# emsig/emg3d

Hardware: AMD Instinct MI355X
Metric: Mcells*smoother-iters/s (fp64) per multigrid cycle (higher is better)
Workload: dtype c128 (complex fp64)

## Files before the change

emg3d_amd/_cycle.py:

```python
import os

import numpy as np
import torch

from emg3d_amd import _lib

__all__ = ['run_cycles', 'coarse_correction', 'coarse_schedule', 'smooth_level', 'stop_reason',
           'ConvergenceError', 'current_sc_dir', 'current_lr_dir']


class ConvergenceError(Exception):
    """Multigrid as preconditioner diverged or stagnated: aborts the Krylov solver."""


def current_sc_dir(sc_dir, grid):
    kept = tuple(n % 2 != 0 or n < 3 or sc_dir == axis + 1 for axis, n in enumerate(grid.shape_cells))
    codes = {(0, 0, 0): 0, (1, 0, 0): 1, (0, 1, 0): 2, (0, 0, 1): 3, (0, 1, 1): 4, (1, 0, 1): 5, (1, 1, 0): 6,
             (1, 1, 1): 6}
    return codes[tuple(int(k) for k in kept)]


_LR_AXES = {0: (), 1: (1,), 2: (2,), 3: (3,), 4: (2, 3), 5: (1, 3), 6: (1, 2), 7: (1, 2, 3)}
_LR_CODE = {axes: code for code, axes in _LR_AXES.items()}

# ... 56 lines not shown
    return budget


class CoarseCorrection:

    def __init__(self, first, first_level, var):
        self.var = var
        self.levels = {first_level: first}

    def run(self, steps):
        var = self.var
        loud = var.verb > 4
        trace = var.first_cycle and var.verb > 3
        sc_at = {}
        for step in steps:
            kind, level = step[0], step[1]
            lv = self.levels[level]
            if kind == SMOOTH:
                smooth_level(lv, step[2], var.lr_dir, var)
                if loud:
                    _log_smoothing(var, level, lv, step[3], step[4], step[5])
            elif kind == DOWN:
                sc_at[level] = current_sc_dir(var.sc_dir, lv.grid)
                lv.residual(store=True, norm=False)
                self.levels[level + 1] = lv.restrict_to(sc_at[level])
            elif kind == UP:
                lv.prolong_from(sc_at[level])
                if trace:
                    var.level_all.append(level)
            elif trace:
                var.level_all.append(level)


def _log_smoothing(var, level, lv, what, it=0, cycmax=None):
    n = lv.grid.shape_cells
    norm = lv.residual(store=False, norm=True)
    visits = var.cycmax if cycmax is None else cycmax
    var.cprint(f"     {it:2} {level} {visits} [{n[0]:3}, {n[1]:3}, {n[2]:3}]: {norm:.3e} {what}", 4)


USE_GRAPHS = os.environ.get('EMG3D_AMD_GRAPHS', '1') != '0'
GRAPH_AFTER = int(os.environ.get('EMG3D_AMD_GRAPH_AFTER', '2'))
CONCURRENT = 0


def coarse_correction(clv, var, budget, first_level=1, graphed=None, top=None):
    depth = int(var.clevel[var.sc_dir])
    steps = coarse_schedule(var.cycle, var.cycmax, depth, first_level, budget, var.nu_pre, var.nu_coarse,
# ... 202 lines not shown
    if leave is not None:
        leave()


def _can_switch(top):
    try:
        top.reserve_residual_equation()
    except torch.cuda.OutOfMemoryError:
        return False
    return True


def _one_cycle(top, var, it, loud):
    if var.clevel[var.sc_dir] == 0:
        smooth_level(top, var.nu_coarse, var.lr_dir, var)
        if loud:
            _log_smoothing(var, 0, top, "coarsest level", it, 1)
        return
    if var.nu_pre > 0:
        smooth_level(top, var.nu_pre, var.lr_dir, var)
        if loud:
            _log_smoothing(var, 0, top, "pre-smoothing", it)
    sc = current_sc_dir(var.sc_dir, top.grid)
    top.residual(store=True, norm=False)
    coarse_correction(top.restrict_to(sc), var, var.cycmax, top=top)
    top.prolong_from(sc)
    if var.first_cycle and var.verb > 3:
        var.level_all.append(0)
    if var.nu_post > 0:
        smooth_level(top, var.nu_post, var.lr_dir, var)
        if loud:
            _log_smoothing(var, 0, top, "post-smoothing", it)


def _level0_visits(var):
    return 1 if var.clevel[var.sc_dir] == 0 else var.cycmax
```

emg3d_amd/_device.py:

```python
import ctypes

import numpy as np
import torch

from emg3d_amd import _lib, meshes
from emg3d_amd import core as _core

_vp = ctypes.c_void_p


def _stream():
    return _vp(torch.cuda.current_stream().cuda_stream)


def _ptr(t, offset_elems=0):
    return _vp(t.data_ptr() + offset_elems * t.element_size())


def coarsen_flags(sc_dir):
    return (sc_dir not in (1, 5, 6), sc_dir not in (2, 4, 6), sc_dir not in (3, 4, 5))


def interp_table(cnodes, nodes):
    i = np.searchsorted(cnodes, nodes) - 1
# ... 388 lines not shown
        for t in tabs:
            pw_slots.append(len(fparts))
            fparts.append(t[1])
        foff = np.cumsum([0] + [a.size for a in fparts])
        fbuf = self.work.upload(np.concatenate(fparts))
        ioff = np.cumsum([0] + [t[0].size for t in tabs])
        ibuf = self.work.upload(np.concatenate([t[0] for t in tabs]))
        wptr = [(_ptr(fbuf, int(foff[i])) if i is not None else None) for i in slots]
        pwptr = [_ptr(fbuf, int(foff[i])) for i in pw_slots]
        ilptr = [_ptr(ibuf, int(ioff[d])) for d in range(3)]
        link = {'level': clevel, 'buffers': (fbuf, ibuf), 'wptr': wptr, 'ilptr': ilptr, 'pwptr': pwptr}
        self.children[sc_dir] = link
        return link

    def restrict_to(self, sc_dir):
        link = self.child(sc_dir)
        c = link['level']
        nx, ny, nz = self.grid.shape_cells
        _lib.check(_lib.lib().emg3d_dev_restrict_clear_batch(
            *c.parts(c.s), *c.parts(c.e), *self.parts(self.r), *link['wptr'], nx, ny, nz, sc_dir,
            self.is_complex, self.batch, self.grid.n_edges, c.grid.n_edges, _stream()), 'emg3d_dev_restrict')
        return c

    def prolong_from(self, sc_dir):
        link = self.children[sc_dir]
        c = link['level']
        nx, ny, nz = self.grid.shape_cells
        _lib.check(_lib.lib().emg3d_dev_prolong_batch(
            *self.parts(self.e), *c.parts(c.e), *link['ilptr'], *link['pwptr'], nx, ny, nz, sc_dir,
            self.is_complex, self.batch, self.grid.n_edges, c.grid.n_edges, _stream()),
            'emg3d_dev_prolong')
```

emg3d_amd/_lib.py:

```python
import ctypes
import os
import subprocess

_HERE = os.path.dirname(os.path.abspath(__file__))
CSRC = os.path.join(_HERE, 'csrc')
LIBDIR = os.path.join(_HERE, 'lib')
LIBPATH = os.path.join(LIBDIR, 'libemg3d_amd.so')
HEADER = os.path.join(os.path.dirname(_HERE), 'include', 'emg3d_amd.h')
SOURCES = [os.path.join(CSRC, f) for f in ('kernels.hip', 'stencil.h', 'launch.h', 'cplx.h', 'receivers.h', 'krylov.h', 'adjoint.h')] + [HEADER]

HIPCC_FLAGS = ['--offload-arch=gfx950', '-O3', '-std=c++17', '-fPIC', '-shared', '-ffp-contract=fast-honor-pragmas']


class Emg3dAmdError(RuntimeError):
    """A C-ABI call returned a non-zero status."""


def build(force=False, verbose=False):
    os.makedirs(LIBDIR, exist_ok=True)
    stale = (not os.path.exists(LIBPATH) or
             any(os.path.getmtime(s) > os.path.getmtime(LIBPATH) for s in SOURCES))
    if force or stale:
        hipcc = os.environ.get('HIPCC', 'hipcc')
        cmd = [hipcc] + HIPCC_FLAGS + [os.path.join(CSRC, 'kernels.hip'), '-o', LIBPATH]
# ... 29 lines not shown
    'emg3d_core_amat_x': (_ci, [_vp] * 13 + [_ci] * 4),
    'emg3d_core_gauss_seidel': (_ci, [_ci] + [_vp] * 13 + [_ci] * 5),
    'emg3d_core_restrict': (_ci, [_vp] * 15 + [_ci] * 5),
    'emg3d_core_blocks_to_amat': (_ci, [_vp] * 5 + [_ci] * 4),
    'emg3d_core_solve': (_ci, [_vp, _vp, _ci, _ci]),
    'emg3d_gs_scratch_bytes': (_sz, [_ci] * 5),
    'emg3d_line_fac_bytes': (_sz, [_ci] * 5),
    'emg3d_line_fac_bytes_lv': (_sz, [ctypes.POINTER(Level), _ci]),
    'emg3d_line_compact_used': (_ci, [ctypes.POINTER(Level), _ci]),
    'emg3d_point_compact_used': (_ci, [ctypes.POINTER(Level)]),
    'emg3d_line_lfac_bytes': (_sz, [_ci] * 4),
    'emg3d_dev_line_setup': (_ci, [ctypes.POINTER(Level), _ci, _vp, _vp, _vp]),
    'emg3d_point_fac_bytes': (_sz, [_ci] * 4),
    'emg3d_point_fac_bytes_lv': (_sz, [ctypes.POINTER(Level)]),
    'emg3d_dev_eta_is_imaginary': (_ci, [ctypes.POINTER(Level), ctypes.POINTER(_ci), _vp]),
    'emg3d_dev_point_setup': (_ci, [ctypes.POINTER(Level), _vp, _vp]),
    'emg3d_dev_gauss_seidel': (_ci, [ctypes.POINTER(Level), _ci, _ci, _vp, _vp, _vp, _sz, _vp]),
    'emg3d_residual_ws_len': (_sz, [_ci] * 3),
    'emg3d_dev_residual': (_ci, [ctypes.POINTER(Level), _vp, _vp, _vp, _vp, _sz, _vp, _vp]),
    'emg3d_dev_restrict': (_ci, [_vp] * 15 + [_ci] * 5 + [_vp]),
    'emg3d_dev_prolong': (_ci, [_vp] * 12 + [_ci] * 5 + [_vp]),
    'emg3d_dev_restrict_batch': (_ci, [_vp] * 15 + [_ci] * 6 + [_sz, _sz, _vp]),
    'emg3d_dev_restrict_clear_batch': (_ci, [_vp] * 18 + [_ci] * 6 + [_sz, _sz, _vp]),
    'emg3d_dev_prolong_batch': (_ci, [_vp] * 12 + [_ci] * 6 + [_sz, _sz, _vp]),
    'emg3d_dev_restrict_param': (_ci, [_vp, _vp] + [_ci] * 5 + [_vp]),
    'emg3d_dev_pec_zero': (_ci, [_vp] * 3 + [_ci] * 4 + [_vp]),
    'emg3d_krylov_ws_len': (_sz, []),
    'emg3d_dev_krylov_step': (_ci, [_sz, _ci, _vp, _ci, _vp, _vp, _vp, _ci, _vp, _vp, _vp, _ci, _vp, _vp, _vp, _sz, _vp]),
    'emg3d_dev_apply_operator': (_ci, [ctypes.POINTER(Level), _vp, _vp, _vp, _vp]),
    'emg3d_dev_zero': (_ci, [_vp, _sz, _vp]),
    'emg3d_dev_copy': (_ci, [_vp, _vp, _sz, _vp]),
    'emg3d_dev_gradient_accumulate': (_ci, [_ci] * 4 + [_vp] * 6 + [ctypes.c_double] * 2 + [_vp] * 5),
    'emg3d_dev_source_field': (_ci, [_ci] * 4 + [_vp] * 7 + [_ci] + [ctypes.c_double] * 2 + [_vp] * 4),
    'emg3d_dev_volume_model': (_ci, [_ci] * 4 + [_vp] * 5 + [_ci] + [_vp] * 3 + [ctypes.c_double] * 4 + [_vp] * 5),
    'emg3d_dev_magnetic_field': (_ci, [_ci] * 4 + [_vp] * 7 + [ctypes.c_double] * 2 + [_vp] * 4),
    'emg3d_dev_spline_filter': (_ci, [_vp] + [_ci] * 4 + [_vp]),
    'emg3d_dev_spline_eval': (_ci, [_vp] + [_ci] * 4 + [_vp, _ci, _vp, _vp]),
    'emg3d_dev_linear_eval': (_ci, [_vp] + [_ci] * 4 + [_vp, _vp, _ci, _vp, _vp]),
    'emg3d_dev_volume_average': (_ci, [_vp] + [_ci] * 3 + [_vp] * 10 + [_ci] * 3 + [_vp, _ci, _vp]),
}

LEVEL_ETA_IMAG = 1
LEVEL_LINE_COMPACT = 2
LEVEL_POINT_COMPACT = 4

_lib = None
# ... 43 lines not shown
```

emg3d_amd/csrc/kernels.hip:

```cpp
#include <hip/hip_runtime.h>

#include <algorithm>
#include <cstdio>
#include <cstdlib>
#include <cstring>
#include <string>
#include <type_traits>

#include "../../include/emg3d_amd.h"
#include "launch.h"

using emg::cplx;

namespace {

thread_local std::string g_err;

int fail(int code, const char *what)
{
    g_err = what;
    return code;
}

int hipfail(hipError_t e, const char *where)
// ... 20 lines not shown
    L.batch = lv->batch > 1 ? lv->batch : 1;
    L.bstride = lv->batch > 1 ? (size_t)lv->batch_stride : 0;
    L.flags = lv->flags;
    return L;
}

using emg::cdiv;
using emg::cnt_par;
using emg::sc_flags;
using emg::ScDirs;

inline dim3 d3(emg::Dim3 d) { return dim3(d.x, d.y, d.z); }

int g_point_slab = 0;
int g_point_tile_min = 1 << 20;
int g_line_fuse = 2;
int g_line_fuse_max = 1 << 30;
int g_skip_repeat = 1;
int g_tile_fuse = 1;
int g_line_lds = 1;
int g_point_prefetch = 0;
int g_residual_zb = 8;
int g_residual_roll = 1;
int g_line_occ2 = 0;
int g_point_small = 512;
int g_line_lpw = 0;
int g_line_stream = 2;
int g_line_order = 1;
int g_line_stream_r = 0;
int g_line_stream_bmin = 64;
int g_line_stream_lf = 1;
int g_line_wide = 33;
int g_line_wide_bt = 0;
int g_line_debug = 0;
int g_line_compact = 0;
int g_line_compact_rd = 0;
int g_line_compact_colour = 1;
constexpr int LS_PROD_COMPACT = 384;

template <class T> bool pst_stored_half(int flags);
template <> bool pst_stored_half<double>(int) { return true; }
template <> bool pst_stored_half<cplx>(int flags) { return (flags & emg::LEVEL_ETA_IMAG) != 0; }
int g_point_compact = 0;
template <class T> int pst_mode(int flags)
{
    const bool compact = g_point_compact > 0 || (g_point_compact == 0 && (flags & emg::LEVEL_POINT_COMPACT));
// ... 1383 lines not shown
    out += blockIdx.x;
    __shared__ double sm[256];
    double acc = 0.0;
    for (int i = threadIdx.x; i < n; i += 256) acc += partial[i];
    sm[threadIdx.x] = acc;
    __syncthreads();
    for (int s = 128; s > 0; s >>= 1) {
        if ((int)threadIdx.x < s) sm[threadIdx.x] += sm[threadIdx.x + s];
        __syncthreads();
    }
    if (threadIdx.x == 0) *out = sm[0];
}

template <class T> __global__ __launch_bounds__(256) void k_restrict(emg::Restrict<T> R)
{
    const int cix = blockIdx.x * blockDim.x + threadIdx.x;
    const int ciy = blockIdx.y * blockDim.y + threadIdx.y;
    const int b = blockIdx.z / R.cnzn, ciz = blockIdx.z - b * R.cnzn;
    if (cix >= R.cnxn || ciy >= R.cnyn) return;
    R.rx += b * R.fstride; R.ry += b * R.fstride; R.rz += b * R.fstride;
    R.crx += b * R.cstride; R.cry += b * R.cstride; R.crz += b * R.cstride;
    if (R.cex) { R.cex += b * R.cstride; R.cey += b * R.cstride; R.cez += b * R.cstride; }
    emg::restrict_node<T>(R, cix, ciy, ciz);
}

template <class T> __global__ __launch_bounds__(256) void k_prolong(emg::Prolong<T> P)
{
    const int ix = blockIdx.x * blockDim.x + threadIdx.x;
    const int iy = blockIdx.y * blockDim.y + threadIdx.y;
    const int b = blockIdx.z / (P.nz + 1), iz = blockIdx.z - b * (P.nz + 1);
    if (ix > P.nx || iy > P.ny) return;
    P.ex += b * P.fstride; P.ey += b * P.fstride; P.ez += b * P.fstride;
    P.cex += b * P.cstride; P.cey += b * P.cstride; P.cez += b * P.cstride;
    emg::prolong_cell<T>(P, ix, iy, iz);
}

template <class T>
__global__ __launch_bounds__(256) void k_restrict_param(T *out, const T *in, int nx, int ny, int cnx,
                                                        int cny, int fx, int fy, int fz)
{
    const int cix = blockIdx.x * blockDim.x + threadIdx.x;
    const int ciy = blockIdx.y * blockDim.y + threadIdx.y;
    const int ciz = blockIdx.z;
    if (cix >= cnx || ciy >= cny) return;
    emg::restrict_param_cell<T>(out, in, nx, ny, cnx, cny, fx, fy, fz, cix, ciy, ciz);
}
// ... 435 lines not shown
    if (sumsq) hipLaunchKernelGGL(k_reduce_sum, dim3(L.batch), dim3(256), 0, st, ws, (int)nblk, sumsq);
    HIP_TRY(hipGetLastError());
    return 0;
}

template <class T>
int launch_restrict(void *crx, void *cry, void *crz, const void *rx, const void *ry, const void *rz,
                    const double *const w[9], int nx, int ny, int nz, int sc_dir, hipStream_t st, int batch = 1,
                    size_t fstride = 0, size_t cstride = 0, void *cex = nullptr, void *cey = nullptr, void *cez = nullptr)
{
    const ScDirs f = sc_flags(sc_dir);
    if ((f.cx && nx % 2) || (f.cy && ny % 2) || (f.cz && nz % 2))
        return fail(EMG3D_ERR_BADARG, "restrict: odd cell count in a coarsened direction");
    emg::Restrict<T> R = emg::make_restrict<T>(crx, cry, crz, rx, ry, rz, w, nx, ny, nz, sc_dir);
    R.batch = batch > 1 ? batch : 1; R.fstride = fstride; R.cstride = cstride;
    R.cex = (T *)cex; R.cey = (T *)cey; R.cez = (T *)cez;
    const emg::Dim3 g = emg::cell_grid(R.cnxn, R.cnyn, R.cnzn);
    hipLaunchKernelGGL(k_restrict<T>, dim3(g.x, g.y, g.z * R.batch), d3(emg::cell_block()), 0, st, R);
    HIP_TRY(hipGetLastError());
    return 0;
}

template <class T>
int launch_prolong(void *ex, void *ey, void *ez, const void *cex, const void *cey, const void *cez,
                   const int32_t *ilx, const int32_t *ily, const int32_t *ilz, const double *wx,
                   const double *wy, const double *wz, int nx, int ny, int nz, int sc_dir, hipStream_t st,
                   int batch = 1, size_t fstride = 0, size_t cstride = 0)
{
    emg::Prolong<T> P =
        emg::make_prolong<T>(ex, ey, ez, cex, cey, cez, ilx, ily, ilz, wx, wy, wz, nx, ny, nz, sc_dir);
    P.batch = batch > 1 ? batch : 1; P.fstride = fstride; P.cstride = cstride;
    const emg::Dim3 g = emg::cell_grid(nx + 1, ny + 1, nz + 1);
    hipLaunchKernelGGL(k_prolong<T>, dim3(g.x, g.y, g.z * P.batch), d3(emg::cell_block()), 0, st, P);
    HIP_TRY(hipGetLastError());
    return 0;
}

template <class T>
int launch_restrict_param(void *out, const void *in, int nx, int ny, int nz, int sc_dir, hipStream_t st)
{
    const ScDirs f = sc_flags(sc_dir);
    const int fx = f.cx ? 2 : 1, fy = f.cy ? 2 : 1, fz = f.cz ? 2 : 1;
    const int cnx = nx / fx, cny = ny / fy, cnz = nz / fz;
    const dim3 block = d3(emg::cell_block());
    const dim3 grid = d3(emg::cell_grid(cnx, cny, cnz));
    hipLaunchKernelGGL(k_restrict_param<T>, grid, block, 0, st, (T *)out, (const T *)in, nx, ny, cnx, cny, fx, fy, fz);
    HIP_TRY(hipGetLastError());
    return 0;
}


struct DevBuf {
    void *d = nullptr;
    size_t bytes = 0;
    ~DevBuf() { if (d) (void)hipFree(d); }
    hipError_t up(const void *h, size_t n)
// ... 49 lines not shown
    hipError_t e = b.up(tmp, sizeof(double) * (size_t)n);
    delete[] tmp;
    return e;
}

}

extern "C" {

int emg3d_version(void) { return EMG3D_AMD_VERSION; }
const char *emg3d_last_error(void) { return g_err.c_str(); }

struct OptionEntry { const char *name; int *value; };
static const OptionEntry g_options[] = {
    {"point_slab", &g_point_slab},       {"point_tile_min", &g_point_tile_min}, {"line_fuse", &g_line_fuse},
    {"line_fuse_max", &g_line_fuse_max}, {"skip_repeat", &g_skip_repeat},       {"tile_fuse", &g_tile_fuse},
    {"line_lds", &g_line_lds},           {"point_prefetch", &g_point_prefetch}, {"residual_zb", &g_residual_zb},
    {"line_occ2", &g_line_occ2},         {"point_small", &g_point_small},       {"line_lpw", &g_line_lpw},
    {"line_debug", &g_line_debug},       {"line_stream", &g_line_stream},       {"line_stream_r", &g_line_stream_r},
    {"line_order", &g_line_order},       {"point_order", &emg::point_order_ref()},
    {"line_stream_bmin", &g_line_stream_bmin}, {"line_stream_lf", &g_line_stream_lf}, {"residual_roll", &g_residual_roll},
    {"line_wide", &g_line_wide},         {"line_wide_bt", &g_line_wide_bt},     {"line_compact", &g_line_compact},
    {"line_compact_rd", &g_line_compact_rd}, {"point_compact", &g_point_compact},
    {"line_compact_colour", &g_line_compact_colour},
};
constexpr int N_OPTIONS = sizeof(g_options) / sizeof(g_options[0]);
static int g_options_generation = 0;

int emg3d_option_count(void) { return N_OPTIONS; }
const char *emg3d_option_name(int i) { return (i >= 0 && i < N_OPTIONS) ? g_options[i].name : nullptr; }

int emg3d_set_option(const char *name, int value)
{
    if (!name) return fail(EMG3D_ERR_BADARG, "set_option: null name");
    if (!std::strcmp(name, "residual_zb") && value < 1) value = 1;
    if (!std::strcmp(name, "line_lpw") && value != 0 && value != 4 && value != 8 && value != 16 && value != 32)
        return fail(EMG3D_ERR_BADARG, "line_lpw: 0, 4, 8, 16 or 32");
    if (!std::strcmp(name, "line_debug") && value != 0 && !std::getenv("EMG3D_AMD_ALLOW_DEBUG"))
        return fail(EMG3D_ERR_BADARG, "line_debug: wrong results by design; set EMG3D_AMD_ALLOW_DEBUG=1 to use it");
    if (!std::strcmp(name, "line_stream_r") && value != 0 && (value < 4 || value > 32 || value % emg::LINE_PAD != 0))
        return fail(EMG3D_ERR_BADARG, "line_stream_r: 0 (= 16) or a multiple of 4 in 4..32");
    if (!std::strcmp(name, "line_wide") && (value < 0 || value > emg::WIDE_N0_MAX)) return fail(EMG3D_ERR_BADARG, "line_wide: 0 .. 64");
    if (!std::strcmp(name, "line_wide_bt") && value != 0 && value != 192 && value != 256) return fail(EMG3D_ERR_BADARG, "line_wide_bt: 0, 192 or 256");
    if (!std::strcmp(name, "line_compact_rd") && value != 0 && value != 4 && value != 8) return fail(EMG3D_ERR_BADARG, "line_compact_rd: 0, 4 or 8");
    if (!std::strcmp(name, "point_compact") && (value < -1 || value > 1)) return fail(EMG3D_ERR_BADARG, "point_compact: -1, 0 or 1");
    if (!std::strcmp(name, "line_compact") && (value < -1 || value > 1)) return fail(EMG3D_ERR_BADARG, "line_compact: -1, 0 or 1");
    if (!std::strcmp(name, "line_order") && (value < 0 || value > 2)) return fail(EMG3D_ERR_BADARG, "line_order: 0, 1 or 2");
    if (!std::strcmp(name, "point_order") && (value < 0 || value > 1)) return fail(EMG3D_ERR_BADARG, "point_order: 0 or 1");
    for (const OptionEntry &o : g_options)
        if (!std::strcmp(name, o.name)) {
            if (*o.value != value) ++g_options_generation;
            *o.value = value;
            return 0;
        }
    return fail(EMG3D_ERR_BADARG, "set_option: unknown option");
}

int emg3d_options_generation(void) { return g_options_generation; }

#ifdef EMG_WIDE_STAMPS
int emg3d_debug_wide_stamps(unsigned long long *out)
{
    return (int)hipMemcpyFromSymbol(out, HIP_SYMBOL(g_wide_stamps), sizeof(unsigned long long) * 32);
}
#endif

const char *emg3d_line_kernel_name(int lr, int nx, int ny, int nz, int is_complex, int batch)
{
    if (lr < 1 || lr > 3 || nx < 2 || ny < 2 || nz < 2) return "";
    const emg::LineClass lc = emg::line_class(lr - 1, nx, ny, nz, 3);
    if (lc.lines <= 0) return "";
// ... 199 lines not shown
{
    if (sc_dir < 0 || sc_dir > 6) return fail(EMG3D_ERR_BADARG, "restrict: sc_dir must be 0..6");
    const double *const w[9] = {wxl, wx0, wxr, wyl, wy0, wyr, wzl, wz0, wzr};
    return is_complex ? launch_restrict<cplx>(crx, cry, crz, rx, ry, rz, w, nx, ny, nz, sc_dir, (hipStream_t)stream, batch,
                                              fine_stride, coarse_stride)
                      : launch_restrict<double>(crx, cry, crz, rx, ry, rz, w, nx, ny, nz, sc_dir, (hipStream_t)stream,
                                                batch, fine_stride, coarse_stride);
}

int emg3d_dev_restrict_clear_batch(void *crx, void *cry, void *crz, void *cex, void *cey, void *cez, const void *rx,
                                   const void *ry, const void *rz, const double *wxl, const double *wx0,
                                   const double *wxr, const double *wyl, const double *wy0, const double *wyr,
                                   const double *wzl, const double *wz0, const double *wzr, int nx, int ny, int nz,
                                   int sc_dir, int is_complex, int batch, size_t fine_stride, size_t coarse_stride,
                                   void *stream)
{
    if (sc_dir < 0 || sc_dir > 6) return fail(EMG3D_ERR_BADARG, "restrict: sc_dir must be 0..6");
    if (!cex || !cey || !cez) return fail(EMG3D_ERR_BADARG, "restrict_clear: coarse field missing");
    const double *const w[9] = {wxl, wx0, wxr, wyl, wy0, wyr, wzl, wz0, wzr};
    return is_complex ? launch_restrict<cplx>(crx, cry, crz, rx, ry, rz, w, nx, ny, nz, sc_dir, (hipStream_t)stream, batch,
                                              fine_stride, coarse_stride, cex, cey, cez)
                      : launch_restrict<double>(crx, cry, crz, rx, ry, rz, w, nx, ny, nz, sc_dir, (hipStream_t)stream,
                                                batch, fine_stride, coarse_stride, cex, cey, cez);
}

int emg3d_dev_prolong_batch(void *ex, void *ey, void *ez, const void *cex, const void *cey, const void *cez,
                            const int32_t *ilx, const int32_t *ily, const int32_t *ilz, const double *wx,
                            const double *wy, const double *wz, int nx, int ny, int nz, int sc_dir, int is_complex,
                            int batch, size_t fine_stride, size_t coarse_stride, void *stream)
{
    if (sc_dir < 0 || sc_dir > 6) return fail(EMG3D_ERR_BADARG, "prolong: sc_dir must be 0..6");
    return is_complex ? launch_prolong<cplx>(ex, ey, ez, cex, cey, cez, ilx, ily, ilz, wx, wy, wz, nx, ny, nz, sc_dir,
                                             (hipStream_t)stream, batch, fine_stride, coarse_stride)
                      : launch_prolong<double>(ex, ey, ez, cex, cey, cez, ilx, ily, ilz, wx, wy, wz, nx, ny, nz, sc_dir,
                                               (hipStream_t)stream, batch, fine_stride, coarse_stride);
}

int emg3d_dev_restrict_param(void *out, const void *in, int nx, int ny, int nz, int sc_dir, int is_complex,
                             void *stream)
{
    if (sc_dir < 0 || sc_dir > 6) return fail(EMG3D_ERR_BADARG, "restrict_param: sc_dir must be 0..6");
    return is_complex ? launch_restrict_param<cplx>(out, in, nx, ny, nz, sc_dir, (hipStream_t)stream)
                      : launch_restrict_param<double>(out, in, nx, ny, nz, sc_dir, (hipStream_t)stream);
}

int emg3d_dev_pec_zero(void *ex, void *ey, void *ez, int nx, int ny, int nz, int is_complex, void *stream)
// ... 157 lines not shown
```

emg3d_amd/csrc/stencil.h:

```cpp
#pragma once
#include "cplx.h"

namespace emg {

template <class T> struct Level {
    int nx, ny, nz;
    T *ex, *ey, *ez;
    const T *sx, *sy, *sz;
    const T *eta_x, *eta_y, *eta_z;
    const double *zeta;
    const double *ihx, *ihy, *ihz;
    int batch = 1;
    size_t bstride = 0;
    int flags = 0;
};
constexpr int LEVEL_ETA_IMAG = 1;
constexpr int LEVEL_LINE_COMPACT = 2;
constexpr int LEVEL_POINT_COMPACT = 4;
template <class T> EMG_HD Level<T> source_level(Level<T> L, int b)
{
    size_t o = (size_t)b * L.bstride;
#if defined(__HIP_DEVICE_COMPILE__)
    o = ((size_t)__builtin_amdgcn_readfirstlane((unsigned)(o >> 32)) << 32) | (size_t)__builtin_amdgcn_readfirstlane((unsigned)o);
#endif
// ... 1421 lines not shown
        getT(b.k, Tk);
        wide_x<T, 15>(Tk, c[b.k], gh[b.k], x);
        wide_block_scatter<T, DIR>(A, b.k, b.mir, i1, i2, x);
    }
    {
        const T xs[5] = {xq[0], xq[1], xq[2], xq[3], xq[4]};
        wide_block_scatter<T, DIR>(A, mk, 0, i1, i2, xs);
        A.E(0)[A.idx(0, mk + 1, i1, i2)] = xq[5];
    }
}

template <class T> struct Restrict {
    int cx, cy, cz;
    int nxn, nyn, nzn;
    int cnxn, cnyn, cnzn;
    const T *rx, *ry, *rz;
    T *crx, *cry, *crz;
    T *cex = nullptr, *cey = nullptr, *cez = nullptr;
    const double *wx[3], *wy[3], *wz[3];
    int batch = 1;
    size_t fstride = 0, cstride = 0;
};

template <class T> EMG_HD void restrict_node(const Restrict<T> &R, int cix, int ciy, int ciz)
{
    const int nx = R.nxn, ny = R.nyn, nz = R.nzn;
    const int cnx = R.cnxn, cny = R.cnyn;
    const int ix = R.cx ? 2 * cix : cix, iy = R.cy ? 2 * ciy : ciy, iz = R.cz ? 2 * ciz : ciz;
    int ixs[3], iys[3], izs[3];
    double wxs[3], wys[3], wzs[3];
    ixs[0] = ix; ixs[1] = ix > 0 ? ix - 1 : 0; ixs[2] = ix + 1 < nx - 1 ? ix + 1 : nx - 1;
    iys[0] = iy; iys[1] = iy > 0 ? iy - 1 : 0; iys[2] = iy + 1 < ny - 1 ? iy + 1 : ny - 1;
    izs[0] = iz; izs[1] = iz > 0 ? iz - 1 : 0; izs[2] = iz + 1 < nz - 1 ? iz + 1 : nz - 1;
    wxs[0] = R.cx ? R.wx[1][cix] : 1.0; wxs[1] = R.cx ? R.wx[0][cix] : 0.0; wxs[2] = R.cx ? R.wx[2][cix] : 0.0;
    wys[0] = R.cy ? R.wy[1][ciy] : 1.0; wys[1] = R.cy ? R.wy[0][ciy] : 0.0; wys[2] = R.cy ? R.wy[2][ciy] : 0.0;
    wzs[0] = R.cz ? R.wz[1][ciz] : 1.0; wzs[1] = R.cz ? R.wz[0][ciz] : 0.0; wzs[2] = R.cz ? R.wz[2][ciz] : 0.0;
    const int nxt = R.cx ? 3 : 1, nyt = R.cy ? 3 : 1, nzt = R.cz ? 3 : 1;

    if (cix < cnx - 1) {
        T acc = zero<T>();
        for (int a = 0; a < nyt; ++a) {
            T inner = zero<T>();
            for (int b = 0; b < nzt; ++b) {
                T v = R.rx[ix + (nx - 1) * (iys[a] + ny * izs[b])];
                if (R.cx) v += R.rx[ixs[2] + (nx - 1) * (iys[a] + ny * izs[b])];
                inner += wzs[b] * v;
            }
            acc += wys[a] * inner;
        }
        R.crx[cix + (cnx - 1) * (ciy + cny * ciz)] = acc;
        if (R.cex) R.cex[cix + (cnx - 1) * (ciy + cny * ciz)] = zero<T>();
    }
    if (ciy < cny - 1) {
        T acc = zero<T>();
        for (int a = 0; a < nxt; ++a) {
            T inner = zero<T>();
            for (int b = 0; b < nzt; ++b) {
                T v = R.ry[ixs[a] + nx * (iy + (ny - 1) * izs[b])];
                if (R.cy) v += R.ry[ixs[a] + nx * (iys[2] + (ny - 1) * izs[b])];
                inner += wzs[b] * v;
            }
            acc += wxs[a] * inner;
        }
        R.cry[cix + cnx * (ciy + (cny - 1) * ciz)] = acc;
        if (R.cey) R.cey[cix + cnx * (ciy + (cny - 1) * ciz)] = zero<T>();
    }
    if (ciz < R.cnzn - 1) {
        T acc = zero<T>();
        for (int a = 0; a < nxt; ++a) {
            T inner = zero<T>();
            for (int b = 0; b < nyt; ++b) {
                T v = R.rz[ixs[a] + nx * (iys[b] + ny * iz)];
                if (R.cz) v += R.rz[ixs[a] + nx * (iys[b] + ny * izs[2])];
                inner += wys[b] * v;
            }
            acc += wxs[a] * inner;
        }
        R.crz[cix + cnx * (ciy + cny * ciz)] = acc;
        if (R.cez) R.cez[cix + cnx * (ciy + cny * ciz)] = zero<T>();
    }
}

template <class T> struct Prolong {
    int cx, cy, cz;
    int nx, ny, nz;
    int cnx, cny, cnz;
    T *ex, *ey, *ez;
    const T *cex, *cey, *cez;
    const int *ilx, *ily, *ilz;
    const double *wx, *wy, *wz;
    int batch = 1;
    size_t fstride = 0, cstride = 0;
};

template <class T> EMG_HD void prolong_cell(const Prolong<T> &P, int ix, int iy, int iz)
{
    const int nx = P.nx, ny = P.ny, nz = P.nz, cnx = P.cnx, cny = P.cny;
    const bool ty = iy >= 1 && iy <= ny - 1, tz = iz >= 1 && iz <= nz - 1, tx = ix >= 1 && ix <= nx - 1;
    if (ix < nx && ty && tz) {
        const int cix = P.cx ? ix / 2 : ix;
        const int a = P.ily[iy], b = P.ilz[iz];
        const double wa = P.wy[iy], wb = P.wz[iz];
        const T *c = P.cex + cix;
        const T v = c[cnx * (a + (cny + 1) * b)] * ((1 - wa) * (1 - wb)) +
// ... 96 lines not shown
```

emg3d_amd/solver.py:

```python
import os

import numpy as np
import torch

from emg3d_amd import _cycle, _lib, fields, models
from emg3d_amd._cycle import ConvergenceError as _ConvergenceError
from emg3d_amd._cycle import current_lr_dir as _current_lr_dir
from emg3d_amd._cycle import current_sc_dir as _current_sc_dir
from emg3d_amd._cycle import one_liner as _print_one_liner
from emg3d_amd._cycle import record_cycle as _print_cycle_info
from emg3d_amd._cycle import smooth_level as _smooth
from emg3d_amd._cycle import terminate as _terminate
from emg3d_amd._device import DeviceLevel
from emg3d_amd._params import MGParameters, Timer

__all__ = ['solve', 'solve_batch', 'solve_source', 'multigrid', 'krylov', 'smoothing', 'restriction',
           'prolongation', 'residual', 'MGParameters', 'RegularGridProlongator']


def __dir__():
    return __all__


_SOLVE_EXTRAS = {'always_return': False, 'plain': False, 'efield': None, 'hierarchy': None,
# ... 273 lines not shown
    if resform:
        lv._b_valid = False
    if getattr(lv, '_resmode', None) is not None:
        lv._resmode = None
    l2_last = lv.residual(store=resform, norm=True)
    l2_stag = np.ones((nb, svar.maxcycle)) * l2_last[:, None]
    active = [True] * nb if active is None else list(active)
    done = [None] * nb
    failed = [False] * nb
    base = [v.smoother_cell_sweeps for v in vars_]
    s0 = svar.smoother_cell_sweeps
    if svar.nu_init > 0:
        _smooth(lv, svar.nu_init, svar.lr_dir, svar)
        if resform:
            lv.residual(store=True, norm=False)
    while any(active):
        l2_prev = l2_last.copy()
        l2_stag[:, (it - 1) % svar.maxcycle] = l2_last
        if resform:
            lv.to_residual_equation()
        if svar.nu_pre > 0:
            _smooth(lv, svar.nu_pre, svar.lr_dir, svar)
        sc_dir = _current_sc_dir(svar.sc_dir, lv.grid)
        lv.residual(store=True, norm=False)
        clv = lv.restrict_to(sc_dir)
        _cycle.coarse_correction(clv, svar, cycmax, top=lv)
        lv.prolong_from(sc_dir)
        if svar.nu_post > 0:
            _smooth(lv, svar.nu_post, svar.lr_dir, svar)
        it += 1
        if resform:
            lv.from_residual_equation()
        l2_last = lv.residual(store=resform, norm=True)
        sc_now, lr_now = svar.sc_dir, svar.lr_dir
        if svar.sc_cycle:
            svar.sc_dir = next(svar.sc_cycle)
        if svar.lr_cycle:
            svar.lr_dir = next(svar.lr_cycle)
        switch, stalled = False, []
        for b, v in enumerate(vars_):
            if not active[b]:
                continue
            v.it += 1
            v.smoother_cell_sweeps = base[b] + (svar.smoother_cell_sweeps - s0)
            v.sc_dir, v.lr_dir = sc_now, lr_now
            _print_cycle_info(v, float(l2_last[b]), float(l2_prev[b]))
            v.sc_dir, v.lr_dir = svar.sc_dir, svar.lr_dir
            stag = float(l2_stag[b, (it - 1) % svar.maxcycle])
# ... 361 lines not shown
```

include/emg3d_amd.h:

```cpp
#ifndef EMG3D_AMD_H
#define EMG3D_AMD_H

#include <stddef.h>
#include <stdint.h>

#ifdef __cplusplus
extern "C" {
#endif

#define EMG3D_AMD_VERSION 100

#define EMG3D_ERR_BADARG (-1)
#define EMG3D_ERR_NODEVICE (-2)
#define EMG3D_ERR_SCRATCH (-3)

typedef struct emg3d_level {
    int32_t nx, ny, nz;
    int32_t is_complex;
    void *ex, *ey, *ez;
    const void *sx, *sy, *sz;
    const void *eta_x, *eta_y, *eta_z;
    const double *zeta;
    const double *ihx, *ihy, *ihz;
    int32_t batch;
// ... 63 lines not shown
                       const void *rz, const double *wxl, const double *wx0, const double *wxr,
                       const double *wyl, const double *wy0, const double *wyr, const double *wzl,
                       const double *wz0, const double *wzr, int nx, int ny, int nz, int sc_dir,
                       int is_complex, void *stream);

int emg3d_dev_prolong(void *ex, void *ey, void *ez, const void *cex, const void *cey, const void *cez,
                      const int32_t *ilx, const int32_t *ily, const int32_t *ilz, const double *wx,
                      const double *wy, const double *wz, int nx, int ny, int nz, int sc_dir,
                      int is_complex, void *stream);

int emg3d_dev_restrict_batch(void *crx, void *cry, void *crz, const void *rx, const void *ry,
                             const void *rz, const double *wxl, const double *wx0, const double *wxr,
                             const double *wyl, const double *wy0, const double *wyr, const double *wzl,
                             const double *wz0, const double *wzr, int nx, int ny, int nz, int sc_dir,
                             int is_complex, int batch, size_t fine_stride, size_t coarse_stride,
                             void *stream);
int emg3d_dev_restrict_clear_batch(void *crx, void *cry, void *crz, void *cex, void *cey, void *cez,
                                   const void *rx, const void *ry, const void *rz, const double *wxl,
                                   const double *wx0, const double *wxr, const double *wyl,
                                   const double *wy0, const double *wyr, const double *wzl,
                                   const double *wz0, const double *wzr, int nx, int ny, int nz,
                                   int sc_dir, int is_complex, int batch, size_t fine_stride,
                                   size_t coarse_stride, void *stream);
int emg3d_dev_prolong_batch(void *ex, void *ey, void *ez, const void *cex, const void *cey,
                            const void *cez, const int32_t *ilx, const int32_t *ily, const int32_t *ilz,
                            const double *wx, const double *wy, const double *wz, int nx, int ny, int nz,
                            int sc_dir, int is_complex, int batch, size_t fine_stride,
                            size_t coarse_stride, void *stream);

int emg3d_dev_restrict_param(void *out, const void *in, int nx, int ny, int nz, int sc_dir,
                             int is_complex, void *stream);

int emg3d_dev_pec_zero(void *ex, void *ey, void *ez, int nx, int ny, int nz, int is_complex,
                       void *stream);

size_t emg3d_krylov_ws_len(void);
int emg3d_dev_krylov_step(size_t n, int is_complex, void *y, int nterms, const void *const *xs, const int *slots,
                          const double *scales, int ndots, const void *const *das, const void *const *dbs,
                          const int *dslots, int nprog, const int *prog, double *table, double *ws, size_t ws_len,
                          void *stream);
int emg3d_dev_apply_operator(const emg3d_level *lv, void *ox, void *oy, void *oz, void *stream);
int emg3d_dev_zero(void *p, size_t bytes, void *stream);
int emg3d_dev_copy(void *dst, const void *src, size_t bytes, void *stream);

int emg3d_dev_magnetic_field(int nx, int ny, int nz, int is_complex, const void *ex, const void *ey,
                             const void *ez, const double *zeta, const double *hx, const double *hy,
// ... 37 lines not shown
```

Before: 3866.

## Fuse residual computation with restriction into one tiled LDS kernel

Adds a fused kernel that computes the residual for a fine-grid tile, keeps a three-plane rolling window of it in shared memory, and restricts it straight to the coarse level while clearing the coarse solution. This avoids writing the full fine residual to global memory and reading it back in a separate restrict launch. A host-side heuristic picks the tile shape to fill about twice the compute-unit count, and blocks are remapped across XCDs. It also retunes the prolong block shape to reduce padding. In exchange, residual values at tile halos are recomputed and occupancy is limited by LDS use.

```diff
diff --git a/emg3d_amd/_cycle.py b/emg3d_amd/_cycle.py
--- a/emg3d_amd/_cycle.py
+++ b/emg3d_amd/_cycle.py
@@ -102,8 +102,7 @@
                     _log_smoothing(var, level, lv, step[3], step[4], step[5])
             elif kind == DOWN:
                 sc_at[level] = current_sc_dir(var.sc_dir, lv.grid)
-                lv.residual(store=True, norm=False)
-                self.levels[level + 1] = lv.restrict_to(sc_at[level])
+                self.levels[level + 1] = lv.residual_restrict_to(sc_at[level])
             elif kind == UP:
                 lv.prolong_from(sc_at[level])
                 if trace:
@@ -352,8 +351,7 @@
         if loud:
             _log_smoothing(var, 0, top, "pre-smoothing", it)
     sc = current_sc_dir(var.sc_dir, top.grid)
-    top.residual(store=True, norm=False)
-    coarse_correction(top.restrict_to(sc), var, var.cycmax, top=top)
+    coarse_correction(top.residual_restrict_to(sc), var, var.cycmax, top=top)
     top.prolong_from(sc)
     if var.first_cycle and var.verb > 3:
         var.level_all.append(0)
diff --git a/emg3d_amd/_device.py b/emg3d_amd/_device.py
--- a/emg3d_amd/_device.py
+++ b/emg3d_amd/_device.py
@@ -434,6 +434,20 @@
             self.is_complex, self.batch, self.grid.n_edges, c.grid.n_edges, _stream()), 'emg3d_dev_restrict')
         return c
 
+    def residual_restrict_to(self, sc_dir):
+        lib = _lib.lib()
+        if lib.emg3d_get_option(b'down_fused') != 1:
+            self.residual(store=True, norm=False)
+            return self.restrict_to(sc_dir)
+        link = self.child(sc_dir)
+        c = link['level']
+        cref = self._cref
+        if self.__dict__.get('_resmode') == 'idle':
+            cref = ctypes.byref(self._level_on(self._x_kept, self._b_kept))
+        _lib.check(lib.emg3d_dev_residual_restrict(cref, *c.parts(c.s), *c.parts(c.e), *link['wptr'], sc_dir,
+                                                   c.grid.n_edges, _stream()), 'emg3d_dev_residual_restrict')
+        return c
+
     def prolong_from(self, sc_dir):
         link = self.children[sc_dir]
         c = link['level']
diff --git a/emg3d_amd/_lib.py b/emg3d_amd/_lib.py
--- a/emg3d_amd/_lib.py
+++ b/emg3d_amd/_lib.py
@@ -75,6 +75,7 @@
     'emg3d_dev_prolong': (_ci, [_vp] * 12 + [_ci] * 5 + [_vp]),
     'emg3d_dev_restrict_batch': (_ci, [_vp] * 15 + [_ci] * 6 + [_sz, _sz, _vp]),
     'emg3d_dev_restrict_clear_batch': (_ci, [_vp] * 18 + [_ci] * 6 + [_sz, _sz, _vp]),
+    'emg3d_dev_residual_restrict': (_ci, [ctypes.POINTER(Level)] + [_vp] * 15 + [_ci, _sz, _vp]),
     'emg3d_dev_prolong_batch': (_ci, [_vp] * 12 + [_ci] * 6 + [_sz, _sz, _vp]),
     'emg3d_dev_restrict_param': (_ci, [_vp, _vp] + [_ci] * 5 + [_vp]),
     'emg3d_dev_pec_zero': (_ci, [_vp] * 3 + [_ci] * 4 + [_vp]),
diff --git a/emg3d_amd/csrc/kernels.hip b/emg3d_amd/csrc/kernels.hip
--- a/emg3d_amd/csrc/kernels.hip
+++ b/emg3d_amd/csrc/kernels.hip
@@ -66,6 +66,8 @@
 int g_point_prefetch = 0;
 int g_residual_zb = 8;
 int g_residual_roll = 1;
+int g_down_fused = 1;
+int g_down_tile_x = 0;
 int g_line_occ2 = 0;
 int g_point_small = 512;
 int g_line_lpw = 0;
@@ -1495,6 +1497,57 @@
     R.crx += b * R.cstride; R.cry += b * R.cstride; R.crz += b * R.cstride;
     if (R.cex) { R.cex += b * R.cstride; R.cey += b * R.cstride; R.cez += b * R.cstride; }
     emg::restrict_node<T>(R, cix, ciy, ciz);
+}
+
+constexpr int N_XCD = 8;
+__device__ inline int xcd_item(int bid, int n)
+{
+    const int q = n / N_XCD, r = n % N_XCD, x = bid % N_XCD;
+    return x * q + min(x, r) + bid / N_XCD;
+}
+
+template <class T>
+__global__ __launch_bounds__(256) void k_residual_restrict(emg::Level<T> L0, emg::Restrict<T> R, int tx, int ty,
+                                                           int ntx, int nty, int zb, int nzb, int nf)
+{
+    extern __shared__ __align__(16) unsigned char down_lds[];
+    T *lx = (T *)down_lds, *ly = lx + 3 * nf, *lz = ly + 3 * nf;
+    int item = xcd_item(blockIdx.x, gridDim.x);
+    const int tix = item % ntx; item /= ntx;
+    const int tiy = item % nty; item /= nty;
+    const int zbk = item % nzb, b = item / nzb;
+    const emg::Level<T> L = emg::source_level(L0, b);
+    R.crx += b * R.cstride; R.cry += b * R.cstride; R.crz += b * R.cstride;
+    R.cex += b * R.cstride; R.cey += b * R.cstride; R.cez += b * R.cstride;
+    const emg::DownTile t = emg::down_tile<T>(R, tx, ty, tix, tiy);
+    const emg::RestrictSrcTile<T> src{lx, ly, lz, t.fx0, t.fy0, t.fx, t.fy};
+    const int tid = threadIdx.x;
+    const bool walker = tid < t.fx * t.fy;
+    const int ix = t.fx0 + tid % t.fx, iy = t.fy0 + tid / t.fx;
+    const int ncx = t.cx1 - t.cx0, nc = ncx * (t.cy1 - t.cy0);
+    const int cz0 = zbk * zb, cz1 = min(cz0 + zb, R.cnzn);
+    emg::ResIn<T> in;
+    bool have = false;
+    int last = -1;
+    for (int ciz = cz0; ciz < cz1; ++ciz) {
+        int lo, hi;
+        emg::down_span(ciz, ciz + 1, L.nz, R.cz, lo, hi);
+        if (lo <= last) lo = last + 1;
+        __syncthreads();
+        if (walker)
+            for (int k = lo; k <= hi; ++k) {
+                T ox = emg::zero<T>(), oy = emg::zero<T>(), oz = emg::zero<T>();
+                emg::residual_column_cell<T>(L, in, have, ix, iy, k, ox, oy, oz);
+                const int a = src.at(ix, iy, k);
+                lx[a] = ox; ly[a] = oy; lz[a] = oz;
+            }
+        last = hi;
+        __syncthreads();
+        for (int w = tid; w < 3 * nc; w += blockDim.x) {
+            const int c = w % nc;
+            emg::restrict_node_src<T>(R, src, t.cx0 + c % ncx, t.cy0 + c / ncx, ciz, 1 << (w / nc));
+        }
+    }
 }
 
 template <class T> __global__ __launch_bounds__(256) void k_prolong(emg::Prolong<T> P)
@@ -1976,6 +2029,51 @@
 }
 
 template <class T>
+int launch_residual_restrict(const emg3d_level *lv, void *crx, void *cry, void *crz, void *cex, void *cey, void *cez,
+                             const double *const w[9], int sc_dir, size_t cstride, hipStream_t st)
+{
+    const emg::Level<T> L = to_level<T>(lv);
+    const int nx = L.nx, ny = L.ny, nz = L.nz;
+    const ScDirs f = sc_flags(sc_dir);
+    if ((f.cx && nx % 2) || (f.cy && ny % 2) || (f.cz && nz % 2))
+        return fail(EMG3D_ERR_BADARG, "residual_restrict: odd cell count in a coarsened direction");
+    emg::Restrict<T> R = emg::make_restrict<T>(crx, cry, crz, nullptr, nullptr, nullptr, w, nx, ny, nz, sc_dir);
+    R.batch = L.batch; R.fstride = L.bstride; R.cstride = cstride;
+    R.cex = (T *)cex; R.cey = (T *)cey; R.cez = (T *)cez;
+    const auto span = [](int t, int c, int n) { return c ? std::min(2 * t + 1, n + 1) : t; };
+    const int want = 2 * compute_units();
+    int tx = 1, ty = 1, zb = 1;
+    double best = -1.0;
+    size_t best_blocks = 0;
+    for (int x = 1; x <= R.cnxn; ++x) {
+        if (g_down_tile_x > 0 && x != std::min(g_down_tile_x, R.cnxn)) continue;
+        const int fx = span(x, f.cx, nx);
+        if (fx > 256) break;
+        for (int y = 1; y <= R.cnyn; ++y) {
+            const int fy = span(y, f.cy, ny);
+            if (fx * fy > 256) break;
+            const size_t tiles = (size_t)cdiv(R.cnxn, x) * cdiv(R.cnyn, y) * L.batch;
+            int z = 8;
+            while (z > 1 && tiles * cdiv(R.cnzn, z) < (size_t)want) z /= 2;
+            const size_t blocks = tiles * cdiv(R.cnzn, z);
+            const int planes = f.cz ? std::min(2 * z + 1, nz + 1) : z;
+            const double lines = (double)blocks * planes * (fy + 2) * (cdiv(fx * (int)sizeof(T), 128) + 1);
+            const bool full = blocks >= (size_t)want, best_full = best_blocks >= (size_t)want;
+            if (best < 0.0 || (full && !best_full) || (full == best_full && (full ? lines < best : blocks > best_blocks))) {
+                best = lines; best_blocks = blocks; tx = x; ty = y; zb = z;
+            }
+        }
+    }
+    const int nf = span(tx, f.cx, nx) * span(ty, f.cy, ny);
+    const int ntx = cdiv(R.cnxn, tx), nty = cdiv(R.cnyn, ty), nzb = cdiv(R.cnzn, zb);
+    const size_t lds = (size_t)9 * nf * sizeof(T);
+    hipLaunchKernelGGL(k_residual_restrict<T>, dim3(ntx * nty * nzb * L.batch), dim3(256), lds, st, L, R, tx, ty, ntx, nty,
+                       zb, nzb, nf);
+    HIP_TRY(hipGetLastError());
+    return 0;
+}
+
+template <class T>
 int launch_prolong(void *ex, void *ey, void *ez, const void *cex, const void *cey, const void *cez,
                    const int32_t *ilx, const int32_t *ily, const int32_t *ilz, const double *wx,
                    const double *wy, const double *wz, int nx, int ny, int nz, int sc_dir, hipStream_t st,
@@ -1984,8 +2082,12 @@
     emg::Prolong<T> P =
         emg::make_prolong<T>(ex, ey, ez, cex, cey, cez, ilx, ily, ilz, wx, wy, wz, nx, ny, nz, sc_dir);
     P.batch = batch > 1 ? batch : 1; P.fstride = fstride; P.cstride = cstride;
-    const emg::Dim3 g = emg::cell_grid(nx + 1, ny + 1, nz + 1);
-    hipLaunchKernelGGL(k_prolong<T>, dim3(g.x, g.y, g.z * P.batch), d3(emg::cell_block()), 0, st, P);
+    int bx = 64;
+    for (int c = 32; c >= 16; c /= 2)
+        if ((size_t)cdiv(nx + 1, c) * c * cdiv(ny + 1, 256 / c) * (256 / c) < (size_t)cdiv(nx + 1, bx) * bx * cdiv(ny + 1, 256 / bx) * (256 / bx))
+            bx = c;
+    const dim3 block(bx, 256 / bx, 1), grid(cdiv(nx + 1, bx), cdiv(ny + 1, 256 / bx), (nz + 1) * P.batch);
+    hipLaunchKernelGGL(k_prolong<T>, grid, block, 0, st, P);
     HIP_TRY(hipGetLastError());
     return 0;
 }
@@ -2081,7 +2183,7 @@
     {"line_stream_bmin", &g_line_stream_bmin}, {"line_stream_lf", &g_line_stream_lf}, {"residual_roll", &g_residual_roll},
     {"line_wide", &g_line_wide},         {"line_wide_bt", &g_line_wide_bt},     {"line_compact", &g_line_compact},
     {"line_compact_rd", &g_line_compact_rd}, {"point_compact", &g_point_compact},
-    {"line_compact_colour", &g_line_compact_colour},
+    {"line_compact_colour", &g_line_compact_colour}, {"down_fused", &g_down_fused}, {"down_tile_x", &g_down_tile_x},
 };
 constexpr int N_OPTIONS = sizeof(g_options) / sizeof(g_options[0]);
 static int g_options_generation = 0;
@@ -2106,6 +2208,8 @@
     if (!std::strcmp(name, "line_compact") && (value < -1 || value > 1)) return fail(EMG3D_ERR_BADARG, "line_compact: -1, 0 or 1");
     if (!std::strcmp(name, "line_order") && (value < 0 || value > 2)) return fail(EMG3D_ERR_BADARG, "line_order: 0, 1 or 2");
     if (!std::strcmp(name, "point_order") && (value < 0 || value > 1)) return fail(EMG3D_ERR_BADARG, "point_order: 0 or 1");
+    if (!std::strcmp(name, "down_fused") && (value < 0 || value > 1)) return fail(EMG3D_ERR_BADARG, "down_fused: 0 or 1");
+    if (!std::strcmp(name, "down_tile_x") && value < 0) return fail(EMG3D_ERR_BADARG, "down_tile_x: >= 0");
     for (const OptionEntry &o : g_options)
         if (!std::strcmp(name, o.name)) {
             if (*o.value != value) ++g_options_generation;
@@ -2351,6 +2455,21 @@
                                               fine_stride, coarse_stride, cex, cey, cez)
                       : launch_restrict<double>(crx, cry, crz, rx, ry, rz, w, nx, ny, nz, sc_dir, (hipStream_t)stream,
                                                 batch, fine_stride, coarse_stride, cex, cey, cez);
+}
+
+int emg3d_dev_residual_restrict(const emg3d_level *lv, void *crx, void *cry, void *crz, void *cex, void *cey, void *cez,
+                                const double *wxl, const double *wx0, const double *wxr, const double *wyl,
+                                const double *wy0, const double *wyr, const double *wzl, const double *wz0,
+                                const double *wzr, int sc_dir, size_t coarse_stride, void *stream)
+{
+    if (!lv) return fail(EMG3D_ERR_BADARG, "residual_restrict: bad argument");
+    if (sc_dir < 0 || sc_dir > 6) return fail(EMG3D_ERR_BADARG, "residual_restrict: sc_dir must be 0..6");
+    if (!crx || !cry || !crz || !cex || !cey || !cez) return fail(EMG3D_ERR_BADARG, "residual_restrict: coarse buffer missing");
+    const double *const w[9] = {wxl, wx0, wxr, wyl, wy0, wyr, wzl, wz0, wzr};
+    return lv->is_complex ? launch_residual_restrict<cplx>(lv, crx, cry, crz, cex, cey, cez, w, sc_dir, coarse_stride,
+                                                           (hipStream_t)stream)
+                          : launch_residual_restrict<double>(lv, crx, cry, crz, cex, cey, cez, w, sc_dir, coarse_stride,
+                                                             (hipStream_t)stream);
 }
 
 int emg3d_dev_prolong_batch(void *ex, void *ey, void *ez, const void *cex, const void *cey, const void *cez,
diff --git a/emg3d_amd/csrc/stencil.h b/emg3d_amd/csrc/stencil.h
--- a/emg3d_amd/csrc/stencil.h
+++ b/emg3d_amd/csrc/stencil.h
@@ -1467,7 +1467,16 @@
     size_t fstride = 0, cstride = 0;
 };
 
-template <class T> EMG_HD void restrict_node(const Restrict<T> &R, int cix, int ciy, int ciz)
+template <class T> struct RestrictSrcGlobal {
+    const T *rx, *ry, *rz;
+    int nx, ny;
+    EMG_HD T x(int i, int j, int k) const { return rx[i + (nx - 1) * (j + ny * k)]; }
+    EMG_HD T y(int i, int j, int k) const { return ry[i + nx * (j + (ny - 1) * k)]; }
+    EMG_HD T z(int i, int j, int k) const { return rz[i + nx * (j + ny * k)]; }
+};
+
+template <class T, class Src>
+EMG_HD void restrict_node_src(const Restrict<T> &R, const Src &src, int cix, int ciy, int ciz, int comp = 7)
 {
     const int nx = R.nxn, ny = R.nyn, nz = R.nzn;
     const int cnx = R.cnxn, cny = R.cnyn;
@@ -1482,13 +1491,13 @@
     wzs[0] = R.cz ? R.wz[1][ciz] : 1.0; wzs[1] = R.cz ? R.wz[0][ciz] : 0.0; wzs[2] = R.cz ? R.wz[2][ciz] : 0.0;
     const int nxt = R.cx ? 3 : 1, nyt = R.cy ? 3 : 1, nzt = R.cz ? 3 : 1;
 
-    if (cix < cnx - 1) {
+    if ((comp & 1) && cix < cnx - 1) {
         T acc = zero<T>();
         for (int a = 0; a < nyt; ++a) {
             T inner = zero<T>();
             for (int b = 0; b < nzt; ++b) {
-                T v = R.rx[ix + (nx - 1) * (iys[a] + ny * izs[b])];
-                if (R.cx) v += R.rx[ixs[2] + (nx - 1) * (iys[a] + ny * izs[b])];
+                T v = src.x(ix, iys[a], izs[b]);
+                if (R.cx) v += src.x(ixs[2], iys[a], izs[b]);
                 inner += wzs[b] * v;
             }
             acc += wys[a] * inner;
@@ -1496,13 +1505,13 @@
         R.crx[cix + (cnx - 1) * (ciy + cny * ciz)] = acc;
         if (R.cex) R.cex[cix + (cnx - 1) * (ciy + cny * ciz)] = zero<T>();
     }
-    if (ciy < cny - 1) {
+    if ((comp & 2) && ciy < cny - 1) {
         T acc = zero<T>();
         for (int a = 0; a < nxt; ++a) {
             T inner = zero<T>();
             for (int b = 0; b < nzt; ++b) {
-                T v = R.ry[ixs[a] + nx * (iy + (ny - 1) * izs[b])];
-                if (R.cy) v += R.ry[ixs[a] + nx * (iys[2] + (ny - 1) * izs[b])];
+                T v = src.y(ixs[a], iy, izs[b]);
+                if (R.cy) v += src.y(ixs[a], iys[2], izs[b]);
                 inner += wzs[b] * v;
             }
             acc += wxs[a] * inner;
@@ -1510,13 +1519,13 @@
         R.cry[cix + cnx * (ciy + (cny - 1) * ciz)] = acc;
         if (R.cey) R.cey[cix + cnx * (ciy + (cny - 1) * ciz)] = zero<T>();
     }
-    if (ciz < R.cnzn - 1) {
+    if ((comp & 4) && ciz < R.cnzn - 1) {
         T acc = zero<T>();
         for (int a = 0; a < nxt; ++a) {
             T inner = zero<T>();
             for (int b = 0; b < nyt; ++b) {
-                T v = R.rz[ixs[a] + nx * (iys[b] + ny * iz)];
-                if (R.cz) v += R.rz[ixs[a] + nx * (iys[b] + ny * izs[2])];
+                T v = src.z(ixs[a], iys[b], iz);
+                if (R.cz) v += src.z(ixs[a], iys[b], izs[2]);
                 inner += wys[b] * v;
             }
             acc += wxs[a] * inner;
@@ -1525,6 +1534,60 @@
         if (R.cez) R.cez[cix + cnx * (ciy + cny * ciz)] = zero<T>();
     }
 }
+
+template <class T> EMG_HD void restrict_node(const Restrict<T> &R, int cix, int ciy, int ciz)
+{
+    const RestrictSrcGlobal<T> src{R.rx, R.ry, R.rz, R.nxn, R.nyn};
+    restrict_node_src<T>(R, src, cix, ciy, ciz);
+}
+
+struct DownTile {
+    int cx0, cx1, cy0, cy1;
+    int fx0, fy0, fx, fy;
+};
+
+EMG_HD void down_span(int c0, int c1, int n, int coarsened, int &f0, int &f1)
+{
+    f0 = coarsened ? (2 * c0 - 1 > 0 ? 2 * c0 - 1 : 0) : c0;
+    f1 = coarsened ? (2 * c1 - 1 < n ? 2 * c1 - 1 : n) : c1 - 1;
+}
+
+template <class T> EMG_HD DownTile down_tile(const Restrict<T> &R, int tx, int ty, int tix, int tiy)
+{
+    DownTile t;
+    t.cx0 = tix * tx; t.cx1 = t.cx0 + tx < R.cnxn ? t.cx0 + tx : R.cnxn;
+    t.cy0 = tiy * ty; t.cy1 = t.cy0 + ty < R.cnyn ? t.cy0 + ty : R.cnyn;
+    int f1;
+    down_span(t.cx0, t.cx1, R.nxn - 1, R.cx, t.fx0, f1); t.fx = f1 - t.fx0 + 1;
+    down_span(t.cy0, t.cy1, R.nyn - 1, R.cy, t.fy0, f1); t.fy = f1 - t.fy0 + 1;
+    return t;
+}
+
+template <class T>
+EMG_HD void residual_column_cell(const Level<T> &L, ResIn<T> &in, bool &have, int ix, int iy, int iz, T &ox, T &oy, T &oz)
+{
+    const Axes<T, 0> A(L);
+    if (ix < L.nx && iy < L.ny && iz < L.nz) {
+        if (have) residual_load_roll<T>(L, ix, iy, iz, in);
+        else residual_load<T>(L, ix, iy, iz, in);
+        have = true;
+        residual_compute<T, true>(L, in, ix, iy, iz, ox, oy, oz);
+    } else {
+        have = false;
+        if (ix < L.nx) ox = L.sx[A.iex(ix, iy, iz)];
+        if (iy < L.ny) oy = L.sy[A.iey(ix, iy, iz)];
+        if (iz < L.nz) oz = L.sz[A.iez(ix, iy, iz)];
+    }
+}
+
+template <class T> struct RestrictSrcTile {
+    const T *lx, *ly, *lz;
+    int fx0, fy0, fx, fy;
+    EMG_HD int at(int i, int j, int k) const { return (i - fx0) + fx * ((j - fy0) + fy * (k % 3)); }
+    EMG_HD T x(int i, int j, int k) const { return lx[at(i, j, k)]; }
+    EMG_HD T y(int i, int j, int k) const { return ly[at(i, j, k)]; }
+    EMG_HD T z(int i, int j, int k) const { return lz[at(i, j, k)]; }
+};
 
 template <class T> struct Prolong {
     int cx, cy, cz;
diff --git a/emg3d_amd/solver.py b/emg3d_amd/solver.py
--- a/emg3d_amd/solver.py
+++ b/emg3d_amd/solver.py
@@ -319,8 +319,7 @@
         if svar.nu_pre > 0:
             _smooth(lv, svar.nu_pre, svar.lr_dir, svar)
         sc_dir = _current_sc_dir(svar.sc_dir, lv.grid)
-        lv.residual(store=True, norm=False)
-        clv = lv.restrict_to(sc_dir)
+        clv = lv.residual_restrict_to(sc_dir)
         _cycle.coarse_correction(clv, svar, cycmax, top=lv)
         lv.prolong_from(sc_dir)
         if svar.nu_post > 0:
diff --git a/include/emg3d_amd.h b/include/emg3d_amd.h
--- a/include/emg3d_amd.h
+++ b/include/emg3d_amd.h
@@ -109,6 +109,11 @@
                                    const double *wz0, const double *wzr, int nx, int ny, int nz,
                                    int sc_dir, int is_complex, int batch, size_t fine_stride,
                                    size_t coarse_stride, void *stream);
+int emg3d_dev_residual_restrict(const emg3d_level *lv, void *csx, void *csy, void *csz, void *cex, void *cey,
+                                void *cez, const double *wxl, const double *wx0, const double *wxr,
+                                const double *wyl, const double *wy0, const double *wyr, const double *wzl,
+                                const double *wz0, const double *wzr, int sc_dir, size_t coarse_stride,
+                                void *stream);
 int emg3d_dev_prolong_batch(void *ex, void *ey, void *ez, const void *cex, const void *cey,
                             const void *cez, const int32_t *ilx, const int32_t *ily, const int32_t *ilz,
                             const double *wx, const double *wy, const double *wz, int nx, int ny, int nz,
```

Result: no change. 3874 (median of 6 runs) (+0.2%).
